# chilir/spotter

Hardware: AMD Instinct MI355X
Metric: images/sec RT-DETRv2-R101 640² bs32 at 1/2/4/8 MI355X; p50 /detect latency (higher is better)
Workload: dtype fp32; 1 GPU; RT-DETRv2-r101vd 640x640 batch=32/GPU preprocess+forward+postprocess; model=rtdetr_v2_r101vd, global_batch=32, image_size=640, parallelism=replicas x1

## Files before the change

### include/spotter_hip.h

```cpp
#ifndef SPOTTER_HIP_H
#define SPOTTER_HIP_H

#include <stddef.h>
#include <stdint.h>

#ifdef __cplusplus
extern "C" {
#endif

#define SP_ABI_VERSION 16

enum sp_act { SP_ACT_NONE = 0, SP_ACT_RELU = 1, SP_ACT_SILU = 2, SP_ACT_GELU = 3 };
enum sp_precision { SP_PREC_FP32 = 0, SP_PREC_BF16 = 1, SP_PREC_F32X3 = 2 };

typedef struct {
  const uint8_t* data;
  int32_t height, width;
  int32_t row_stride;
} sp_image_u8;

typedef struct {
  const float* A; int64_t lda;
  const float* A2; int64_t lda2;
  int32_t N, H, W, Cin;
  int32_t KH, KW, stride, pad;
  int32_t Ho, Wo;
  const float* Wt; int32_t Cout;
  const float* scale;
  const float* shift;
  const float* row_scale; int32_t row_period;
  const float* res1; int64_t ldr1;
  int32_t act;
  const float* res2; int64_t ldr2;
  float* C; int64_t ldc;
  int32_t out_rows_per_group; int64_t out_group_stride;
  float* workspace; int64_t workspace_elems;
  int32_t precision;
  const uint16_t* Wt_bf16;
  int64_t wt_plane_stride;
  const float* ln_gamma;
  const float* ln_beta;
  float ln_eps;
  const uint16_t* A_bf16;
  uint16_t* C_bf16;
  const uint16_t* res1_bf16;
  const uint16_t* res2_bf16;
  int32_t* splitk_counters; int64_t splitk_counters_len;
} sp_conv_desc;

typedef struct {
  const float* value; int64_t ld_value; int32_t value_col;
  const float* off_aw; int64_t ld_off_aw;
  const float* ref;
  float* out; int64_t ld_out;
  int32_t B, S, Q, heads, head_dim, levels, points;
  int32_t level_h[4], level_w[4], level_start[4];
  float offset_scale;
  const uint16_t* value_bf16;
} sp_msda_desc;

int sp_abi_version(void);
const char* sp_last_error(void);
enum sp_build_flag { SP_BUILD_FUSED_LN = 1, SP_BUILD_BOUNDS = 2 };
int sp_build_flags(void);
int64_t sp_bounds_report(char* buf, int64_t cap);
int sp_device_init(int device);
int sp_shutdown(void);

int sp_preprocess_u8(const sp_image_u8* images, int n, int out_h, int out_w, float* out,
                     void* stream);

int sp_conv2d(const sp_conv_desc* d, void* stream);
int sp_set_conv_config(int cfg);
int sp_set_splitk_config(int cfg, int max_splits, int min_ktiles);
enum sp_tuning_knob {
  SP_TUNE_GLDS_EPILOGUE = 3,
  SP_TUNE_MSDA_GENERIC = 4,
};
int sp_set_tuning(int knob, int value);

int sp_conv3x3_winograd(const sp_conv_desc* d, const uint16_t* wt_wino, int64_t wino_plane_stride, float* work,
                        int64_t work_elems, void* stream);
int sp_winograd_f23_input(const sp_conv_desc* d, float* work, int64_t work_elems, void* stream);
int sp_winograd_f23_gemm(const sp_conv_desc* d, const uint16_t* wt_wino, int64_t wino_plane_stride, float* work,
                         int64_t work_elems, void* stream);
int sp_winograd_f23_output(const sp_conv_desc* d, const float* work, int64_t work_elems, void* stream);
int sp_winograd_f43_input(const sp_conv_desc* d, float* work, int64_t work_elems, void* stream);
int sp_winograd_f43_gemm(const sp_conv_desc* d, const uint16_t* wt_wino, int64_t wino_plane_stride, float* work,
                         int64_t work_elems, void* stream);
int sp_winograd_f43_output(const sp_conv_desc* d, const float* work, int64_t work_elems, void* stream);

int sp_nchw_to_nhwc(const float* x, float* y, int n, int c, int h, int w, void* stream);
int sp_stem_conv3x3s2_nchw(const float* x, const float* wt, const float* scale, const float* shift, float* y,
                           int n, int h, int w, int cout, int act, void* stream);
int sp_stem_conv3x3s2_nchw_bf16(const float* x, const float* wt, const float* scale, const float* shift, uint16_t* y,
                                int n, int h, int w, int cout, int act, void* stream);
int sp_conv3x3_c32_bf16(const uint16_t* x, const uint16_t* w16, const float* scale, const float* shift, uint16_t* y,
                        int n, int h, int w, int cout, int act, void* stream);
int sp_conv3x3_c32(const float* x, const float* wt, const float* scale, const float* shift, float* y, int n, int h,
                   int w, int cout, int act, void* stream);
int sp_conv3x3_c64_bf16(const uint16_t* x, int64_t ldx, const uint16_t* w16, const float* scale, const float* shift,
                        uint16_t* y, int64_t ldy, const uint16_t* res, int64_t ldr, int n, int h, int w, int act,
                        void* stream);
int sp_maxpool3x3s2(const float* x, float* y, int64_t ldy, int n, int h, int w, int c, void* stream);
int sp_maxpool3x3s2_bf16(const uint16_t* x, uint16_t* y, int64_t ldy, int n, int h, int w, int c, void* stream);
int sp_avgpool2x2_ceil(const float* x, float* y, int64_t ldy, int n, int h, int w, int c, void* stream);
int sp_avgpool2x2_ceil_bf16(const uint16_t* x, uint16_t* y, int64_t ldy, int n, int h, int w, int c, void* stream);
int sp_upsample2x_nearest(const float* x, int64_t ldx, float* y, int64_t ldy, int n, int h,
                          int w, int c, void* stream);
int sp_layernorm(const float* x, int64_t ldx, const float* gamma, const float* beta, float* y,
                 int64_t ldy, int rows, int d, float eps, void* stream);
int sp_layernorm_bf16(const float* x, int64_t ldx, const float* gamma, const float* beta, uint16_t* y, int64_t ldy,
                      int rows, int d, float eps, void* stream);
int sp_attention(const float* q, int64_t ldq, const float* k, int64_t ldk, const float* v,
                 int64_t ldv, float* o, int64_t ldo, int batch, int n, int heads, int dh,
                 float scale, void* stream);
int sp_attention_bf16(const float* q, int64_t ldq, const float* k, int64_t ldk, const float* v,
                      int64_t ldv, float* o, int64_t ldo, int batch, int n, int heads, int dh,
                      float scale, void* stream);
int sp_msda(const sp_msda_desc* d, void* stream);
int sp_topk_rows(const float* x, int64_t ldx, int rows, int n, int reduce_c, int apply_sigmoid,
                 int k, float* vals, int32_t* idx, void* stream);
int sp_rowmax(const float* x, int64_t ldx, int64_t rows, int c, float* out, void* stream);
int sp_linear_rowmax_bf16(const uint16_t* a, int64_t lda, const uint16_t* w, const float* bias, int rows, int n,
                          int k, float* out, void* stream);
int sp_gather_rows(const float* src, int64_t ld_src, int src_rows, const int32_t* idx, int k,
                   int batch, int d, float* dst, int64_t ld_dst, void* stream);
int sp_add_rows(const float* a, int64_t lda, const float* b, int64_t ldb, float* y, uint16_t* y_bf16, int64_t ldy,
                int rows, int cols, void* stream);
int sp_ref_init(const float* delta, int64_t ld_delta, const float* anchors, const int32_t* idx,
                int batch, int k, float* ref, void* stream);
int sp_box_refine(const float* delta, int64_t ld_delta, float* ref, int rows, void* stream);
int sp_postprocess(const float* logits, const float* boxes, const int32_t* target_hw, int batch,
                   int q, int c, int k, float threshold, float* scores, int64_t* labels,
                   float* boxes_xyxy, int32_t* counts, int32_t* work, void* stream);

#define SP_JPEG_UNSUPPORTED (-10)
typedef struct {
  int32_t width, height;
  int32_t ncomp;
  int32_t color;
  int32_t progressive;
  int32_t max_h, max_v;
  int32_t h[3], v[3];
  int32_t bw[3], bh[3];
  int64_t block_off[3];
  int64_t total_blocks;
  int64_t plane_off[3];
  int64_t plane_bytes;
  uint16_t quant[3][64];
} sp_jpeg_layout;
int sp_jpeg_decode_coefs(const uint8_t* data, int64_t len, sp_jpeg_layout* lay, int16_t* coefs, int64_t coef_elems);
int sp_jpeg_to_rgb(const int16_t* coefs, const sp_jpeg_layout* lay, uint8_t* work, int64_t work_bytes, uint8_t* rgb,
                   int64_t rgb_stride, int32_t* status, void* stream);

typedef struct {
// ... 53 lines not shown
```

### spotter_amd/_lib.py

```python
from __future__ import annotations

import ctypes as C
import os
import threading

HERE = os.path.dirname(os.path.abspath(__file__))
LIB_PATH = os.environ.get("SPOTTER_HIP_LIB", os.path.join(HERE, "libspotter_hip.so"))
ABI_VERSION = 16

vp = C.c_void_p
i32 = C.c_int32
i64 = C.c_int64
f32 = C.c_float


class SpImageU8(C.Structure):
    _fields_ = [("data", vp), ("height", i32), ("width", i32), ("row_stride", i32)]


class SpConvDesc(C.Structure):
    _fields_ = [
        ("A", vp), ("lda", i64), ("A2", vp), ("lda2", i64),
        ("N", i32), ("H", i32), ("W", i32), ("Cin", i32),
        ("KH", i32), ("KW", i32), ("stride", i32), ("pad", i32),
        ("Ho", i32), ("Wo", i32),
        ("Wt", vp), ("Cout", i32),
        ("scale", vp), ("shift", vp),
        ("row_scale", vp), ("row_period", i32),
        ("res1", vp), ("ldr1", i64),
        ("act", i32),
        ("res2", vp), ("ldr2", i64),
        ("C", vp), ("ldc", i64),
        ("out_rows_per_group", i32), ("out_group_stride", i64),
        ("workspace", vp), ("workspace_elems", i64),
        ("precision", i32), ("Wt_bf16", vp), ("wt_plane_stride", i64),
        ("ln_gamma", vp), ("ln_beta", vp), ("ln_eps", f32),
        ("A_bf16", vp),
        ("C_bf16", vp), ("res1_bf16", vp), ("res2_bf16", vp),
        ("splitk_counters", vp), ("splitk_counters_len", i64),
    ]


class SpMsdaDesc(C.Structure):
    _fields_ = [
        ("value", vp), ("ld_value", i64), ("value_col", i32),
        ("off_aw", vp), ("ld_off_aw", i64),
        ("ref", vp),
        ("out", vp), ("ld_out", i64),
        ("B", i32), ("S", i32), ("Q", i32), ("heads", i32), ("head_dim", i32),
        ("levels", i32), ("points", i32),
        ("level_h", i32 * 4), ("level_w", i32 * 4), ("level_start", i32 * 4),
        ("offset_scale", f32),
        ("value_bf16", vp),
    ]


class SpJpegLayout(C.Structure):
    _fields_ = [
        ("width", i32), ("height", i32), ("ncomp", i32), ("color", i32), ("progressive", i32),
        ("max_h", i32), ("max_v", i32), ("h", i32 * 3), ("v", i32 * 3), ("bw", i32 * 3), ("bh", i32 * 3),
        ("block_off", i64 * 3), ("total_blocks", i64), ("plane_off", i64 * 3), ("plane_bytes", i64),
# ... 15 lines not shown
    _fields_ = [
        ("kind", i32), ("x0", i32), ("y0", i32), ("x1", i32), ("y1", i32), ("ink", C.c_uint32),
        ("mask_off", i64), ("mask_stride", i32), ("sx", i32), ("sy", i32), ("reserved", i32),
    ]


class SpDrawTile(C.Structure):
    _fields_ = [("tx", i32), ("ty", i32), ("first", i32), ("count", i32)]


class SpDrawTable(C.Structure):
    _fields_ = [
        ("n_ops", i32), ("n_tiles", i32), ("n_refs", i32), ("height", i32), ("width", i32), ("reserved", i32),
        ("ops_off", i64), ("tiles_off", i64), ("refs_off", i64), ("masks_off", i64), ("mask_bytes", i64),
        ("total_bytes", i64),
    ]


SP_DRAW_FILL, SP_DRAW_BLEND = 0, 1
SP_DRAW_TILE_W, SP_DRAW_TILE_H = 64, 8
SP_JPEG_UNSUPPORTED = -10
SP_BUILD_FUSED_LN = 1
SP_BUILD_BOUNDS = 2

_SIGS = {
    "sp_abi_version": (i32, []),
    "sp_build_flags": (i32, []),
    "sp_bounds_report": (i64, [C.c_char_p, i64]),
    "sp_last_error": (C.c_char_p, []),
    "sp_device_init": (i32, [i32]),
    "sp_shutdown": (i32, []),
    "sp_preprocess_u8": (i32, [C.POINTER(SpImageU8), i32, i32, i32, vp, vp]),
    "sp_conv2d": (i32, [C.POINTER(SpConvDesc), vp]),
    "sp_set_conv_config": (i32, [i32]),
    "sp_set_splitk_config": (i32, [i32, i32, i32]),
    "sp_set_tuning": (i32, [i32, i32]),
    "sp_conv3x3_winograd": (i32, [C.POINTER(SpConvDesc), vp, i64, vp, i64, vp]),
    "sp_winograd_f23_input": (i32, [C.POINTER(SpConvDesc), vp, i64, vp]),
    "sp_winograd_f23_gemm": (i32, [C.POINTER(SpConvDesc), vp, i64, vp, i64, vp]),
    "sp_winograd_f23_output": (i32, [C.POINTER(SpConvDesc), vp, i64, vp]),
    "sp_winograd_f43_input": (i32, [C.POINTER(SpConvDesc), vp, i64, vp]),
    "sp_winograd_f43_gemm": (i32, [C.POINTER(SpConvDesc), vp, i64, vp, i64, vp]),
    "sp_winograd_f43_output": (i32, [C.POINTER(SpConvDesc), vp, i64, vp]),
    "sp_nchw_to_nhwc": (i32, [vp, vp, i32, i32, i32, i32, vp]),
    "sp_stem_conv3x3s2_nchw": (i32, [vp, vp, vp, vp, vp, i32, i32, i32, i32, i32, vp]),
    "sp_maxpool3x3s2": (i32, [vp, vp, i64, i32, i32, i32, i32, vp]),
    "sp_avgpool2x2_ceil": (i32, [vp, vp, i64, i32, i32, i32, i32, vp]),
    "sp_maxpool3x3s2_bf16": (i32, [vp, vp, i64, i32, i32, i32, i32, vp]),
    "sp_avgpool2x2_ceil_bf16": (i32, [vp, vp, i64, i32, i32, i32, i32, vp]),
    "sp_stem_conv3x3s2_nchw_bf16": (i32, [vp, vp, vp, vp, vp, i32, i32, i32, i32, i32, vp]),
    "sp_conv3x3_c32_bf16": (i32, [vp, vp, vp, vp, vp, i32, i32, i32, i32, i32, vp]),
    "sp_conv3x3_c32": (i32, [vp, vp, vp, vp, vp, i32, i32, i32, i32, i32, vp]),
    "sp_conv3x3_c64_bf16": (i32, [vp, i64, vp, vp, vp, vp, i64, vp, i64, i32, i32, i32, i32, vp]),
    "sp_upsample2x_nearest": (i32, [vp, i64, vp, i64, i32, i32, i32, i32, vp]),
    "sp_layernorm": (i32, [vp, i64, vp, vp, vp, i64, i32, i32, f32, vp]),
    "sp_layernorm_bf16": (i32, [vp, i64, vp, vp, vp, i64, i32, i32, f32, vp]),
    "sp_attention": (i32, [vp, i64, vp, i64, vp, i64, vp, i64, i32, i32, i32, i32, f32, vp]),
    "sp_attention_bf16": (i32, [vp, i64, vp, i64, vp, i64, vp, i64, i32, i32, i32, i32, f32, vp]),
    "sp_msda": (i32, [C.POINTER(SpMsdaDesc), vp]),
    "sp_topk_rows": (i32, [vp, i64, i32, i32, i32, i32, i32, vp, vp, vp]),
    "sp_rowmax": (i32, [vp, i64, i64, i32, vp, vp]),
    "sp_gather_rows": (i32, [vp, i64, i32, vp, i32, i32, i32, vp, i64, vp]),
    "sp_ref_init": (i32, [vp, i64, vp, vp, i32, i32, vp, vp]),
    "sp_box_refine": (i32, [vp, i64, vp, i32, vp]),
    "sp_add_rows": (i32, [vp, i64, vp, i64, vp, vp, i64, i32, i32, vp]),
    "sp_linear_rowmax_bf16": (i32, [vp, i64, vp, vp, i32, i32, i32, vp, vp]),
    "sp_postprocess": (i32, [vp, vp, vp, i32, i32, i32, i32, f32, vp, vp, vp, vp, vp, vp]),
    "sp_jpeg_decode_coefs": (i32, [vp, i64, C.POINTER(SpJpegLayout), vp, i64]),
    "sp_jpeg_to_rgb": (i32, [vp, C.POINTER(SpJpegLayout), vp, i64, vp, i64, vp, vp]),
    "sp_jpeg_enc_plan": (i32, [i32, i32, i32, i32, C.POINTER(SpJpegEncLayout)]),
    "sp_jpeg_enc_rgb": (i32, [vp, i64, i32, C.POINTER(SpJpegEncLayout), vp, i64, vp, i64, vp, vp]),
    "sp_jpeg_enc_max_bytes": (i64, [C.POINTER(SpJpegEncLayout), i64, i64]),
    "sp_jpeg_enc_finish": (i32, [C.POINTER(SpJpegEncLayout), vp, i64, vp, i64, vp, i64, C.POINTER(i64)]),
    "sp_draw_pack": (i32, [vp, i32, vp, i64, i32, i32, vp, i64, C.POINTER(i64)]),
    "sp_draw_rgb": (i32, [vp, i32, i32, i64, vp, vp, i64, vp]),
}

EXPORTS = tuple(_SIGS)

_lock = threading.Lock()
_lib = None


def load(path: str = LIB_PATH):
    if not os.path.exists(path):
        raise RuntimeError(
            f"libspotter_hip.so not found at {path}; build it with `python -m spotter_amd.build_ext` "
            "(there is no CPU fallback)")
    import torch

    L = C.CDLL(path)
    for name, (res, args) in _SIGS.items():
        fn = getattr(L, name)
        fn.restype = res
        fn.argtypes = args
    if L.sp_abi_version() != ABI_VERSION:
        raise RuntimeError(f"libspotter_hip ABI {L.sp_abi_version()} != {ABI_VERSION}")
    return L


def lib():
    global _lib
    with _lock:
        if _lib is None:
            _lib = load()
        return _lib
# ... 11 lines not shown
```

### spotter_amd/engine.py

```python
from __future__ import annotations

import math

import numpy as np
import torch

from . import ops
from .config import PRECISIONS, SpotterConfig, check_precision
from .ops import V, view
from .weights import backbone_plan


def _t(a, dev):
    return torch.from_numpy(np.ascontiguousarray(a, dtype=np.float32)).to(dev)


bf16_bits = ops.bf16_bits


ATTN_BF16 = True

_X3_FASTER = {(256, 64, False), (256, 1024, True), (1024, 256, True), (512, 256, True), (256, 512, True),
              (288, 256, True), (4, 256, False)}



def _wkw(wq):
    if wq is None:
        return {}
    if wq.dim() == 2 and wq.shape[0] == 3:
        return {"wt_planes": wq}
    return {"wt16": wq}


class ConvW:
    __slots__ = ("w", "cin", "cout", "k", "scale", "shift", "w16", "host", "wino", "mode")

    def __init__(self, w, cin, cout, k, scale, shift, w16=None, host=None, mode="f32"):
        self.w, self.cin, self.cout, self.k, self.scale, self.shift = w, cin, cout, k, scale, shift
        self.w16 = w16
        self.mode = mode
        self.host = host
        self.wino = None


class LinW:
    __slots__ = ("w", "b", "k", "n", "w16", "mode")

    def __init__(self, w, b, k, n, w16=None, mode="f32"):
        self.w, self.b, self.k, self.n = w, b, k, n
        self.w16 = w16
        self.mode = mode


def frozen_bn_affine(p, pre):
    scale = p[pre + ".weight"] * (p[pre + ".running_var"] + np.float32(1e-5)) ** np.float32(-0.5)
    shift = p[pre + ".bias"] - p[pre + ".running_mean"] * scale
    return scale.astype(np.float32), shift.astype(np.float32)


def eval_bn_affine(p, pre, eps=1e-5):
    inv = (p[pre + ".running_var"] + np.float32(eps)) ** np.float32(-0.5)
    scale = p[pre + ".weight"] * inv
    shift = p[pre + ".bias"] - p[pre + ".running_mean"] * scale
    return scale.astype(np.float32), shift.astype(np.float32)


def conv_khwc(w):
    co, ci, k, _ = w.shape
    return np.ascontiguousarray(w.transpose(0, 2, 3, 1).reshape(co, k * k * ci))


def sine_pos_embed(h, w, dim, temperature):
    pd = dim // 4
    omega = 1.0 / temperature ** (np.arange(pd, dtype=np.float64) / pd)
    gh, gw = np.meshgrid(np.arange(h, dtype=np.float64), np.arange(w, dtype=np.float64), indexing="ij")
    eh = np.outer(gh.reshape(-1), omega)
    ew = np.outer(gw.reshape(-1), omega)
    return np.concatenate([np.sin(eh), np.cos(eh), np.sin(ew), np.cos(ew)], 1).astype(np.float32)


def anchors_for(shapes, grid_size=0.05):
    out = []
    f = np.float32
    for lvl, (h, w) in enumerate(shapes):
        gy, gx = np.meshgrid(np.arange(h, dtype=f), np.arange(w, dtype=f), indexing="ij")
        xy = np.stack([gx, gy], -1) + f(0.5)
        xy[..., 0] /= f(w)
        xy[..., 1] /= f(h)
        wh = np.ones_like(xy) * f(grid_size * 2.0 ** lvl)
        out.append(np.concatenate([xy, wh], -1).reshape(h * w, 4))
    a = np.concatenate(out, 0).astype(f)
    valid = ((a > f(1e-2)) & (a < f(1 - 1e-2))).all(-1)
    lg = np.log(a / (f(1) - a)).astype(f)
    lg[~valid] = np.finfo(f).max
    return lg, valid.astype(f)


class Engine:

    def __init__(self, cfg: SpotterConfig, weights: dict, device: str | torch.device = "cuda",
                 fold_repvgg: bool = True, precision: str = "fp32", fuse_shortcut: bool = True,
                 fuse_ln: bool = False, winograd: str | bool = "auto", wino_m: int = 4,
                 bf16_store: bool | None = None, direct_c32: bool = True,
                 direct_c64_bf16: bool = True, splitk_combine: bool = False):
        from ._lib import SP_BUILD_FUSED_LN, lib

        check_precision(precision)
        self.cfg = cfg
        self.fold_repvgg = fold_repvgg
        self.fuse_shortcut = fuse_shortcut
        self.fuse_ln = fuse_ln
        if fuse_ln and PRECISIONS.get(precision, ("", ""))[1] == "bf16":
            raise ValueError(f"fuse_ln=True runs the linears on fp32 weights: not available with precision={precision!r}")
        if fuse_ln and not (lib().sp_build_flags() & SP_BUILD_FUSED_LN):
            raise ValueError("fuse_ln=True needs a diagnostic library with the fused-LayerNorm tiles "
                             "(UNIT=conv_gemm tools/build_diag.sh <name> -DSP_DIAG_KERNELS=1; SPOTTER_HIP_LIB)")
        if winograd is True:
            winograd = "auto"
        if winograd not in (False, None, "auto", "repvgg", "all"):
            raise ValueError("winograd must be False, 'auto', 'repvgg' or 'all'")
        self.winograd = winograd or False
        if wino_m not in (2, 4):
            raise ValueError("wino_m must be 2 (F(2x2,3x3)) or 4 (F(4x4,3x3))")
        self.wino_m = wino_m
        self.precision = precision
        self.act_bb = cfg.hidden_act
        self.act_enc = cfg.activation_function
        self.act_aifi = cfg.encoder_activation_function
        self.act_dec = cfg.decoder_activation_function
        self._conv_mode, self._lin_mode = PRECISIONS[precision]
        self._attn_bf16 = self._lin_mode == "bf16" and ATTN_BF16
        self.bf16_store = (self._conv_mode == "bf16") if bf16_store is None else bool(bf16_store)
        if self.bf16_store and self._conv_mode != "bf16":
            raise ValueError("bf16_store needs a bf16 conv operand mode")
        self.direct_c32 = direct_c32
        self.direct_c64_bf16 = direct_c64_bf16
        self.splitk_combine = splitk_combine
        self.splitk_min_rows = 0
        self.add_rows = True
        self.enc_head_bf16 = True
        self.enc_rowmax_fused = True
        self.dev = torch.device(device)
        if self.dev.type != "cuda":
            raise RuntimeError("spotter_amd runs on an MI355X (gfx950) device only")
        idx = self.dev.index if self.dev.index is not None else torch.cuda.current_device()
        self.dev = torch.device("cuda", idx)
        rc = lib().sp_device_init(idx)
        if rc != 0:
            raise RuntimeError(f"sp_device_init: {lib().sp_last_error().decode()}")
        with torch.cuda.device(self.dev):
            self._pack(weights)
        self._ws = {}
        self._consts = {}
        self._ctxs = {}
        self._outs = {}
        self.microbatches = None
        self.stagger = 1

    def _wq(self, w: np.ndarray, mode: str):
        if mode == "f32":
            return None
        if mode == "bf16":
            return torch.from_numpy(bf16_bits(w).view(np.int16)).to(self.dev)
        return torch.from_numpy(ops.split_bf16x3_host(w)).to(self.dev)

    def _add_wino(self, cw: ConvW):
        if cw.k != 3 or cw.mode == "f32" or cw.cin % 32 or cw.cout % 4 or not self.winograd:
            return cw
        if self.winograd == "auto" and (cw.cin < (self.WINO43_MIN_CIN if self.wino_m == 4 else 256) or cw.mode != "x3"):
            return cw
        u = ops.winograd_weights_host(cw.host.reshape(cw.cout, 3, 3, cw.cin), self.wino_m)
        if cw.mode == "x3":
            cw.wino = torch.from_numpy(ops.split_bf16x3_host(u)).to(self.dev)
        else:
            cw.wino = torch.from_numpy(bf16_bits(u).reshape(1, -1).view(np.int16)).to(self.dev)
        return cw

    def _pick(self, mode: str, cout: int, kdim: int, small_m: bool = False) -> str:
        if mode == "x3" and self.precision == "fp32" and (cout <= 64 or kdim <= 64 or small_m):
            if cout == 64 and kdim >= 576 and not small_m:
                return mode
            if (cout, kdim, small_m) in _X3_FASTER:
                return mode
            return "f32"
        return mode

    def _mk_conv(self, wk, ci, co, k, sc, sh):
        wk = np.ascontiguousarray(wk, dtype=np.float32)
        mode = self._pick(self._conv_mode, co, ci * k * k)
        return ConvW(_t(wk, self.dev), ci, co, k, _t(sc, self.dev), _t(sh, self.dev), self._wq(wk, mode), host=wk,
                     mode=mode)

    def _conv(self, p, conv_key, bn_pre, frozen):
        w = p[conv_key]
        co, ci, k, _ = w.shape
        sc, sh = frozen_bn_affine(p, bn_pre) if frozen else eval_bn_affine(p, bn_pre, self.cfg.batch_norm_eps)
        return self._mk_conv(conv_khwc(w), ci, co, k, sc, sh)

    def _lin(self, p, pre, *more, per_query: bool = False):
        ws = [p[pre + ".weight"]] + [p[m + ".weight"] for m in more]
        bs = [p[pre + ".bias"]] + [p[m + ".bias"] for m in more]
        w = np.ascontiguousarray(np.concatenate(ws, 0))
        b = np.concatenate(bs, 0)
        wd = _t(w, self.dev)
        mode = self._pick(self._lin_mode, w.shape[0], w.shape[1], small_m=per_query and w.shape[0] > 128)
        return LinW(wd, _t(b, self.dev), w.shape[1], w.shape[0], self._wq(w.astype(np.float32), mode), mode=mode)

    def _ln(self, p, pre):
        return (_t(p[pre + ".weight"], self.dev), _t(p[pre + ".bias"], self.dev))

    def _pack(self, p):
        cfg = self.cfg
        bb = "model.backbone.model"
        self.stem = [self._conv(p, f"{bb}.embedder.embedder.{i}.convolution.weight",
                                f"{bb}.embedder.embedder.{i}.normalization", True) for i in range(3)]
        self.blocks = []
        for (s, i, lt, cin, cout, st, sc) in backbone_plan(cfg):
            pre = f"{bb}.encoder.stages.{s}.layers.{i}"
            blk = {"s": s, "i": i, "type": lt, "cin": cin, "cout": cout, "stride": st, "sc": sc}
            if sc == "conv":
                blk["short"] = self._conv(p, pre + ".shortcut.convolution.weight", pre + ".shortcut.normalization", True)
            elif sc == "avgconv":
                blk["short"] = self._conv(p, pre + ".shortcut.1.convolution.weight", pre + ".shortcut.1.normalization", True)
            nl = 3 if lt == "bottleneck" else 2
            blk["layers"] = [self._conv(p, f"{pre}.layer.{j}.convolution.weight", f"{pre}.layer.{j}.normalization", True)
                             for j in range(nl)]
            if self.winograd in ("auto", "all"):
                for j, c in enumerate(blk["layers"]):
                    if c.k == 3 and (st == 1 or (lt != "bottleneck" and j == 1)):
                        self._add_wino(c)
            if self.fuse_shortcut and lt == "bottleneck" and (sc == "avgconv" or (sc == "conv" and st == 1)):
                sk = pre + (".shortcut.1" if sc == "avgconv" else ".shortcut")
                blk["fused"] = self._fused_tail(p, f"{pre}.layer.2", sk, cin)
            self.blocks.append(blk)
        self.in_proj = [self._conv(p, f"model.encoder_input_proj.{l}.0.weight", f"model.encoder_input_proj.{l}.1", False)
                        for l in range(len(cfg.encoder_in_channels))]
        a = "model.encoder.aifi.0.layers.0"
        self.aifi = {
            "qk": self._lin(p, a + ".self_attn.q_proj", a + ".self_attn.k_proj"),
            "v": self._lin(p, a + ".self_attn.v_proj"),
            "o": self._lin(p, a + ".self_attn.o_proj"),
            "ln1": self._ln(p, a + ".self_attn_layer_norm"),
            "fc1": self._lin(p, a + ".mlp.fc1"),
            "fc2": self._lin(p, a + ".mlp.fc2"),
            "ln2": self._ln(p, a + ".final_layer_norm"),
        }
        E = "model.encoder"
        nl = len(cfg.encoder_in_channels)
        self.lateral = [self._conv(p, f"{E}.lateral_convs.{i}.conv.weight", f"{E}.lateral_convs.{i}.norm", False)
                        for i in range(nl - 1)]
        self.down = [self._conv(p, f"{E}.downsample_convs.{i}.conv.weight", f"{E}.downsample_convs.{i}.norm", False)
                     for i in range(nl - 1)]
        self.fpn = [self._csp(p, f"{E}.fpn_blocks.{i}") for i in range(nl - 1)]
        self.pan = [self._csp(p, f"{E}.pan_blocks.{i}") for i in range(nl - 1)]
        self.dec_proj = [self._conv(p, f"model.decoder_input_proj.{l}.0.weight", f"model.decoder_input_proj.{l}.1", False)
                         for l in range(len(cfg.decoder_in_channels))]
        self.enc_output = self._lin(p, "model.enc_output.0")
        self.enc_ln = self._ln(p, "model.enc_output.1")
        self.enc_score = self._lin(p, "model.enc_score_head")
        self.enc_bbox = [self._lin(p, f"model.enc_bbox_head.layers.{i}", per_query=True) for i in range(3)]
        self.qpos = [self._lin(p, f"model.decoder.query_pos_head.layers.{i}", per_query=True) for i in range(2)]
        D = "model.decoder.layers"
        L = cfg.decoder_layers
        self.value_all = self._lin(p, f"{D}.0.encoder_attn.value_proj",
                                   *[f"{D}.{j}.encoder_attn.value_proj" for j in range(1, L)])
        self.dec = []
        for j in range(L):
            q = f"{D}.{j}"
# ... 50 lines not shown
                reps.append((self._conv(p, q + ".conv1.conv.weight", q + ".conv1.norm", False),
                             self._conv(p, q + ".conv2.conv.weight", q + ".conv2.norm", False)))
        c3 = None
        if (pre + ".conv3.conv.weight") in p:
            c3 = self._conv(p, pre + ".conv3.conv.weight", pre + ".conv3.norm", False)
        return {"c12": c12, "hid": w1.shape[0], "reps": reps, "c3": c3}

    def _buf(self, key, *shape, dtype=torch.float32):
        ws = self._ws
        t = ws.get(key)
        n = int(np.prod(shape))
        if t is None or t.numel() < n or t.dtype != dtype:
            t = torch.empty(n, dtype=dtype, device=self.dev)
            ws[key] = t
        return t[:n]

    SPLITK_COUNTERS = 4096

    def _splitk(self) -> dict:
        kw = {"workspace": self._buf("splitk", self.SPLITK_ELEMS)}
        if self.splitk_combine:
            c = self._ws.get("splitk_cnt")
            if c is None:
                c = torch.zeros(self.SPLITK_COUNTERS, dtype=torch.int32, device=self.dev)
                self._ws["splitk_cnt"] = c
            kw["counters"] = c
        return kw

    def _const(self, key, fn):
        c = self._consts.get(key)
        if c is None:
            c = fn()
            self._consts[key] = c
        return c

    SPLITK_ELEMS = 16 << 20
    WINO43_MIN_CIN = 128
    WINO_MIN_PIXELS = 8192
    WINO43_MIN_WORK = 1 << 19

    def _wino_pays(self, pixels: int, cin: int) -> bool:
        if self.wino_m == 4:
            return pixels * cin >= self.WINO43_MIN_WORK and (cin >= self.WINO43_MIN_CIN or self.winograd != "auto")
        return pixels >= self.WINO_MIN_PIXELS

    def _cv(self, x: V, n, h, w, cw: ConvW, stride, out: V, act=None, res1=None, res2=None, **kw):
        pad = cw.k // 2
        if (cw.cin == 64 and cw.cout == 64 and cw.k == 3 and stride == 1 and not kw and res2 is None
                and act in ("relu", None) and n * h * w >= self.C64_MIN_PIXELS):
            rows16 = lambda v: v.ld % 8 == 0 and v.off % 8 == 0
            if (self.direct_c64_bf16 and x.is_bf16 and out.is_bf16 and cw.mode == "bf16" and rows16(x)
                    and rows16(out) and (res1 is None or (res1.is_bf16 and rows16(res1)))):
                return ops.conv3x3_c64_bf16(x, cw.w16, cw.scale, cw.shift, out, n, h, w, act=act, res1=res1)
        if cw.wino is not None and stride == 1 and not kw and not x.is_bf16 and self._wino_pays(n * h * w, cw.cin):
            wm = self.wino_m
            tiles = n * ((h + wm - 1) // wm) * ((w + wm - 1) // wm)
            work = self._buf("wino_work", ops.wino_work_elems(wm, tiles, cw.cin, cw.cout))
            return ops.conv2d(x, n, h, w, cw.cin, cw.w, cw.cout, 3, 1, 1, out, scale=cw.scale, shift=cw.shift,
                              act=act, res1=res1, res2=res2, wino=(cw.wino, work, wm))
        return ops.conv2d(x, n, h, w, cw.cin, cw.w, cw.cout, cw.k, stride, pad, out, scale=cw.scale,
                          shift=cw.shift, act=act, res1=res1, res2=res2,
                          **self._splitk(), **_wkw(cw.w16), **kw)

    def _lin_op(self, x: V, rows, lw: LinW, out: V, act=None, res1=None, res2=None, a2=None, row_scale=None,
                ln=None):
        if ln is not None and self.fuse_ln:
            if act is not None or res2 is not None:
                raise ValueError("fused LayerNorm epilogue: act / res2 are not implemented")
            if lw.mode == "bf16":
                raise ValueError("fuse_ln runs fp32 weights: not available on a bf16-operand layer")
            return ops.linear(x, rows, lw.k, lw.w, lw.n, out, bias=lw.b, res1=res1, a2=a2, row_scale=row_scale,
                              ln=(ln[0], ln[1], self.cfg.layer_norm_eps))
        if ln is not None:
            tmp = view(self._buf("ln_tmp", rows, lw.n), lw.n)
            ops.linear(x, rows, lw.k, lw.w, lw.n, tmp, bias=lw.b, act=act, res1=res1, res2=res2, a2=a2,
                       row_scale=row_scale, **self._splitk(), **_wkw(lw.w16))
            return ops.layernorm(tmp, *ln, out, rows, lw.n, self.cfg.layer_norm_eps)
        sk = self._splitk() if rows > self.splitk_min_rows else {}
        return ops.linear(x, rows, lw.k, lw.w, lw.n, out, bias=lw.b, act=act, res1=res1, res2=res2, a2=a2,
                          row_scale=row_scale, **sk, **_wkw(lw.w16))

    def _lin_plus(self, x: V, addend: V | None, rows, lw: LinW, out: V, key: str):
        if addend is None:
            return self._lin_op(x, rows, lw, out)
        if not self.add_rows or lw.mode == "f32":
            return self._lin_op(x, rows, lw, out, a2=addend)
        hp = view(self._buf(key, rows, lw.k, dtype=torch.int16 if lw.mode == "bf16" else torch.float32), lw.k)
        ops.add_rows(x, addend, hp, rows, lw.k)
        return self._lin_op(hp, rows, lw, out)

    C64_MIN_PIXELS = 1 << 18
    C32_MIN_PIXELS = 1 << 19

    def _direct_stem(self) -> bool:
        c = self.stem[0]
        return c.cin == 3 and c.k == 3 and c.cout in (32, 64) and self.act_bb in ("relu", None)

    def backbone(self, pixel_values: torch.Tensor, B, H, W):
        e = self.cfg.embedding_size
        h1, w1 = (H - 1) // 2 + 1, (W - 1) // 2 + 1
        dt = torch.int16 if self.bf16_store else torch.float32

        def buf(key, *shape):
            return self._buf(key, *shape, dtype=dt)

        s0 = buf("stem0", B, h1, w1, e // 2)
        s1 = buf("stem1", B, h1, w1, e // 2)
        s2 = buf("stem2", B, h1, w1, e)
        c0 = self.stem[0]
        if self._direct_stem():
            ops.stem_conv_nchw(pixel_values, c0.w, c0.scale, c0.shift, view(s0, e // 2), c0.cout, act=self.act_bb)
        else:
            px = self._buf("px_nhwc", B, H, W, 3)
            ops.nchw_to_nhwc(pixel_values, px)
            self._cv(view(px, 3), B, H, W, c0, 2, view(s0, e // 2), act=self.act_bb)
        for src, cw, dst in ((s0, self.stem[1], s1), (s1, self.stem[2], s2)):
            c32 = cw.cin == 32 and cw.k == 3 and cw.cout in (32, 64) and self.act_bb in ("relu", None)
            if c32 and self.bf16_store:
                ops.conv3x3_c32_bf16(view(src, cw.cin), cw.w16, cw.scale, cw.shift, view(dst, cw.cout), B, h1, w1,
                                     cw.cout, act=self.act_bb)
            elif (c32 and self.direct_c32 and cw.mode == "f32" and not self.bf16_store
                  and B * h1 * w1 >= self.C32_MIN_PIXELS):
                ops.conv3x3_c32(view(src, cw.cin), cw.w, cw.scale, cw.shift, view(dst, cw.cout), B, h1, w1, cw.cout,
                                act=self.act_bb)
            else:
                self._cv(view(src, cw.cin), B, h1, w1, cw, 1, view(dst, cw.cout), act=self.act_bb)
        h, w = (h1 - 1) // 2 + 1, (w1 - 1) // 2 + 1
        b0 = self.blocks[0]
        if "fused" in b0 and b0["sc"] == "conv":
            kc = b0["layers"][0].cout + e
            curv = V(buf(f"s{b0['s']}_cat", B, h, w, kc), kc - e, kc)
        else:
            curv = view(buf("pool", B, h, w, e), e)
        ops.maxpool3x3s2(s2, curv, B, h1, w1, e)
        c = e
        feats = []
        nstage = len(self.cfg.depths)
        for blk in self.blocks:
            s, i, st, cout = blk["s"], blk["i"], blk["stride"], blk["cout"]
            cur = curv.t
            if i == 0 and s > 0:
                assert curv.off == 0 and curv.ld == c
                feats.append((cur, h, w, c))
            ho, wo = (h - 1) // st + 1, (w - 1) // st + 1
            L = blk["layers"]
            if "fused" in blk:
                red = L[0].cout
                kc = red + c
                if blk["sc"] == "avgconv":
                    assert curv.off == 0 and curv.ld == c
                    cat = buf(f"s{s}_cat", B, ho, wo, kc)
                    ops.avgpool2x2_ceil(cur, V(cat, red, kc), B, h, w, c)
                else:
                    assert curv.off == red and curv.ld == kc and st == 1
                    cat = cur
                t1 = buf(f"s{s}_t1", B, h, w, red)
                out = buf(f"s{s}_out{i % 2}", B, ho, wo, cout)
                self._cv(curv, B, h, w, L[0], 1, view(t1, red), act=self.act_bb)
                self._cv(view(t1, red), B, h, w, L[1], st, V(cat, 0, kc), act=self.act_bb)
                self._cv(V(cat, 0, kc), B, ho, wo, blk["fused"], 1, view(out, cout), act=self.act_bb)
                curv, h, w, c = view(out, cout), ho, wo, cout
                yield
                continue
            if blk["sc"] == "identity":
                res = view(cur, c)
            else:
                src, sh_, sw_ = cur, h, w
                if blk["sc"] == "avgconv":
                    pooled = buf(f"s{s}_pool", B, (h + 1) // 2, (w + 1) // 2, c)
                    ops.avgpool2x2_ceil(cur, pooled, B, h, w, c)
                    src, sh_, sw_ = pooled, (h + 1) // 2, (w + 1) // 2
                sbuf = buf(f"s{s}_sc", B, ho, wo, cout)
                self._cv(view(src, c), B, sh_, sw_, blk["short"], 1 if blk["sc"] == "avgconv" else st, view(sbuf, cout))
# ... 279 lines not shown
```

### spotter_amd/ops.py

```python
from __future__ import annotations

import ctypes as C
from dataclasses import dataclass

import numpy as np
import torch

from ._lib import SpConvDesc, SpImageU8, SpMsdaDesc, call

ACT = {None: 0, "none": 0, "relu": 1, "silu": 2, "gelu": 3}

_hook = None


def set_launch_hook(hook):
    global _hook
    _hook = hook


def _launch(kind: str, name: str, args, flops: int = 0, nbytes: int = 0, shape=None):
    if _hook is None:
        call(name, *args)
    else:
        _hook(kind, lambda: call(name, *args), flops, nbytes, shape)
# ... 263 lines not shown
            (x.data_ptr(), wt.data_ptr(), scale.data_ptr(), shift.data_ptr(), yp, n, h, w, cout, ACT[act],
             stream()), 2 * m * cout * 27, 4 * (x.numel() + cout * 27) + y.t.element_size() * m * cout,
            (m, cout, 27, 3, 2, "direct"))
    return ho, wo


def conv3x3_c32_bf16(x: V, w16: torch.Tensor, scale: torch.Tensor, shift: torch.Tensor, y: V, n: int, h: int,
                     w: int, cout: int, act=None):
    if not (x.is_bf16 and y.is_bf16) or x.ld != 32 or y.ld != cout or x.off % 8 or y.off % 8:
        raise ValueError("conv3x3_c32_bf16: dense bf16 rows (ld 32 in, Cout out) expected")
    if w16.dtype != torch.int16 or w16.numel() != cout * 288 or scale.numel() < cout or shift.numel() < cout:
        raise ValueError("conv3x3_c32_bf16: weight / affine size mismatch")
    m = n * h * w
    xp = x.need(m, 32, "c32.x", bf16=True)
    yp = y.need(m, cout, "c32.y", bf16=True)
    _launch("conv", "sp_conv3x3_c32_bf16", (xp, w16.data_ptr(), scale.data_ptr(), shift.data_ptr(), yp, n, h, w,
                                            cout, ACT[act], stream()),
            2 * m * cout * 288, 2 * (m * 32 + cout * 288 + m * cout), (m, cout, 288, 3, 1, "bf16-direct"))


def conv3x3_c32(x: V, wt: torch.Tensor, scale: torch.Tensor, shift: torch.Tensor, y: V, n: int, h: int, w: int,
                cout: int, act=None):
    if x.is_bf16 or y.is_bf16 or x.ld != 32 or y.ld != cout:
        raise ValueError("conv3x3_c32: dense fp32 rows (ld 32 in, Cout out) expected")
    if wt.dtype != torch.float32 or wt.numel() != cout * 288 or scale.numel() < cout or shift.numel() < cout:
        raise ValueError("conv3x3_c32: weight / affine size mismatch")
    m = n * h * w
    xp = x.need(m, 32, "c32.x")
    yp = y.need(m, cout, "c32.y")
    _launch("conv", "sp_conv3x3_c32", (xp, wt.data_ptr(), scale.data_ptr(), shift.data_ptr(), yp, n, h, w, cout,
                                       ACT[act], stream()),
            2 * m * cout * 288, 4 * (m * 32 + cout * 288 + m * cout), (m, cout, 288, 3, 1, "f32-direct"))


def conv3x3_c64_bf16(x: V, w16: torch.Tensor, scale: torch.Tensor, shift: torch.Tensor, y: V, n: int, h: int,
                     w: int, act=None, res1: V | None = None):
    if not (x.is_bf16 and y.is_bf16) or x.ld % 8 or x.off % 8 or y.ld % 8 or y.off % 8:
        raise ValueError("conv3x3_c64_bf16: 16-byte aligned bf16 row views expected")
    if w16.dtype != torch.int16 or w16.numel() != 64 * 576 or scale.numel() < 64 or shift.numel() < 64:
        raise ValueError("conv3x3_c64_bf16: weight / affine size mismatch")
    m = n * h * w
    xp = x.need(m, 64, "c64b.x", bf16=True)
    yp = y.need(m, 64, "c64b.y", bf16=True)
    rp, ldr = None, 0
    if res1 is not None:
        if not res1.is_bf16 or res1.ld % 8 or res1.off % 8:
            raise ValueError("conv3x3_c64_bf16: the residual must be 16-byte aligned bf16 rows")
        rp, ldr = res1.need(m, 64, "c64b.res", bf16=True), res1.ld
    _launch("conv", "sp_conv3x3_c64_bf16", (xp, x.ld, w16.data_ptr(), scale.data_ptr(), shift.data_ptr(), yp, y.ld,
                                            rp, ldr, n, h, w, ACT[act], stream()),
            2 * m * 64 * 576, 2 * (m * 64 + 64 * 576 + m * 64 * (2 if rp else 1)), (m, 64, 576, 3, 1, "bf16-direct"))


def _pool_out(y, m: int, c: int, what: str):
    if isinstance(y, V):
        if y.ld % 4 or y.off % 4 or (y.is_bf16 and (y.ld % 8 or y.off % 8)):
            raise ValueError(f"{what}: output view must be 16-byte aligned")
        return y.need(m, c, what, bf16=y.is_bf16), y.ld
    if y.numel() < m * c:
        raise ValueError(f"{what}: output too small")
    return y.data_ptr(), c


def _pool(name, x: torch.Tensor, y, n, h, w, c, ho, wo):
    assert x.numel() >= n * h * w * c
    bf = x.dtype == torch.int16
    yv = y if isinstance(y, V) else view(y, c)
    if yv.is_bf16 != bf:
        raise TypeError(f"{name}: input and output rows must both be float32 or both bf16")
    yp, ldy = _pool_out(y, n * ho * wo, c, name + ".y")
    _launch("elementwise", name + ("_bf16" if bf else ""), (x.data_ptr(), yp, ldy, n, h, w, c, stream()), 0,
            x.element_size() * n * c * (h * w + ho * wo))
    return ho, wo


def maxpool3x3s2(x: torch.Tensor, y, n, h, w, c):
    return _pool("sp_maxpool3x3s2", x, y, n, h, w, c, (h - 1) // 2 + 1, (w - 1) // 2 + 1)


def avgpool2x2_ceil(x: torch.Tensor, y, n, h, w, c):
    return _pool("sp_avgpool2x2_ceil", x, y, n, h, w, c, (h + 1) // 2, (w + 1) // 2)


def upsample2x(x: V, y: V, n, h, w, c):
    bf = x.is_bf16
    if y.is_bf16 != bf:
        raise TypeError("upsample: input and output rows must both be float32 or both bf16")
    xp = x.need(n * h * w, c, "upsample.x", bf16=bf)
    yp = y.need(n * 4 * h * w, c, "upsample.y", bf16=bf)
    if bf and (c % 8 or x.ld % 2 or y.ld % 2 or x.off % 2 or y.off % 2):
        raise ValueError("upsample: bf16 rows need c % 8 == 0 and even strides / offsets")
    k = 2 if bf else 1
    _launch("elementwise", "sp_upsample2x_nearest", (xp, x.ld // k, yp, y.ld // k, n, h, w, c // k, stream()), 0,
            x.t.element_size() * n * h * w * c * 5)


def layernorm(x: V, gamma, beta, y: V, rows, d, eps=1e-5):
    xp = x.need(rows, d, "ln.x")
    yp = y.need(rows, d, "ln.y", bf16=y.is_bf16)
    _launch("layernorm", "sp_layernorm_bf16" if y.is_bf16 else "sp_layernorm",
            (xp, x.ld, gamma.data_ptr(), beta.data_ptr(), yp, y.ld, rows, d, eps, stream()), 8 * rows * d,
            (4 + y.t.element_size()) * rows * d)


def attention(q: V, k: V, v: V, o: V, batch, n, heads, dh, scale, bf16: bool = False):
    rows = batch * n
# ... 117 lines not shown
```

Baseline: 810.3 images/sec.

## Add direct 3x3 conv kernels using split-bf16x3 MFMA for fp32 c64/c32 layers

Adds a direct (implicit-GEMM) 3x3 conv kernel that splits fp32 activations into three bf16 planes in LDS and runs six bf16 MFMA products per fragment to emulate fp32 accuracy. It tiles 8x32 output pixels with a halo, double-buffers weights with async global-to-LDS loads, and prefetches the next tile's halo into registers. The 64-channel variant is enabled by default for x3-mode convs without a residual, replacing the previous GEMM or Winograd path. The 32-channel stem variant is behind a flag that is off by default. It trades im2col and workspace traffic for extra MFMA work and a persistent grid of one block per CU, and the x3 split approximates fp32 rather than matching it exactly.

```diff
diff --git a/include/spotter_hip.h b/include/spotter_hip.h
--- a/include/spotter_hip.h
+++ b/include/spotter_hip.h
@@ -8,7 +8,7 @@
 extern "C" {
 #endif
 
-#define SP_ABI_VERSION 16
+#define SP_ABI_VERSION 17
 
 enum sp_act { SP_ACT_NONE = 0, SP_ACT_RELU = 1, SP_ACT_SILU = 2, SP_ACT_GELU = 3 };
 enum sp_precision { SP_PREC_FP32 = 0, SP_PREC_BF16 = 1, SP_PREC_F32X3 = 2 };
@@ -102,6 +102,10 @@
 int sp_conv3x3_c64_bf16(const uint16_t* x, int64_t ldx, const uint16_t* w16, const float* scale, const float* shift,
                         uint16_t* y, int64_t ldy, const uint16_t* res, int64_t ldr, int n, int h, int w, int act,
                         void* stream);
+int sp_conv3x3_c64_x3(const float* x, int64_t ldx, const uint16_t* w_planes, int64_t plane_stride, const float* scale,
+                      const float* shift, float* y, int64_t ldy, int n, int h, int w, int act, void* stream);
+int sp_conv3x3_c32_x3(const float* x, const uint16_t* w_planes, int64_t plane_stride, const float* scale,
+                      const float* shift, float* y, int n, int h, int w, int cout, int act, void* stream);
 int sp_maxpool3x3s2(const float* x, float* y, int64_t ldy, int n, int h, int w, int c, void* stream);
 int sp_maxpool3x3s2_bf16(const uint16_t* x, uint16_t* y, int64_t ldy, int n, int h, int w, int c, void* stream);
 int sp_avgpool2x2_ceil(const float* x, float* y, int64_t ldy, int n, int h, int w, int c, void* stream);
diff --git a/spotter_amd/_lib.py b/spotter_amd/_lib.py
--- a/spotter_amd/_lib.py
+++ b/spotter_amd/_lib.py
@@ -6,7 +6,7 @@
 
 HERE = os.path.dirname(os.path.abspath(__file__))
 LIB_PATH = os.environ.get("SPOTTER_HIP_LIB", os.path.join(HERE, "libspotter_hip.so"))
-ABI_VERSION = 16
+ABI_VERSION = 17
 
 vp = C.c_void_p
 i32 = C.c_int32
@@ -128,6 +128,8 @@
     "sp_conv3x3_c32_bf16": (i32, [vp, vp, vp, vp, vp, i32, i32, i32, i32, i32, vp]),
     "sp_conv3x3_c32": (i32, [vp, vp, vp, vp, vp, i32, i32, i32, i32, i32, vp]),
     "sp_conv3x3_c64_bf16": (i32, [vp, i64, vp, vp, vp, vp, i64, vp, i64, i32, i32, i32, i32, vp]),
+    "sp_conv3x3_c64_x3": (i32, [vp, i64, vp, i64, vp, vp, vp, i64, i32, i32, i32, i32, vp]),
+    "sp_conv3x3_c32_x3": (i32, [vp, vp, i64, vp, vp, vp, i32, i32, i32, i32, i32, vp]),
     "sp_upsample2x_nearest": (i32, [vp, i64, vp, i64, i32, i32, i32, i32, vp]),
     "sp_layernorm": (i32, [vp, i64, vp, vp, vp, i64, i32, i32, f32, vp]),
     "sp_layernorm_bf16": (i32, [vp, i64, vp, vp, vp, i64, i32, i32, f32, vp]),
diff --git a/spotter_amd/csrc/direct_x3.hip b/spotter_amd/csrc/direct_x3.hip
--- /dev/null
+++ b/spotter_amd/csrc/direct_x3.hip
@@ -0,0 +1,214 @@
+#include "mfma16_common.h"
+
+namespace sp {
+namespace {
+
+constexpr int DX_TH = 8, DX_TW = 32, DX_HR = DX_TH + 2, DX_HC = DX_TW + 2, DX_NPX = DX_HR * DX_HC;
+
+template <int CIN, int CO, bool RES>
+__global__ __launch_bounds__(512, 1) void conv3x3_x3_kernel(const float* __restrict__ x,
+                                                            const uint16_t* __restrict__ wp, int64_t wps,
+                                                            const float* __restrict__ scale,
+                                                            const float* __restrict__ shift, float* __restrict__ y,
+                                                            int64_t ldx, int64_t ldy, int nimg, int h, int w,
+                                                            int tiles_x, int tiles_y, int act) {
+  constexpr int CPP = CIN / 8;
+  constexpr int PLANE = DX_NPX * CPP;
+  constexpr int SPT = CIN / 32;
+  constexpr int NST = 9 * SPT;
+  constexpr int WPL = CO * 4;
+  constexpr int WST = 3 * WPL;
+  constexpr int NBUF = RES ? NST : 2;
+  constexpr int WDMA = WST / 64;
+  constexpr int TMN = CO / 32;
+  constexpr int PFN = (PLANE + 511) / 512;
+  __shared__ uint4 lds[3 * PLANE + NBUF * WST];
+  __shared__ float aff[2 * CO];
+  uint4* halo = lds;
+  uint4* wl = lds + 3 * PLANE;
+  const int tid = threadIdx.x, lane = tid & 63;
+  const int wave = __builtin_amdgcn_readfirstlane(tid >> 6);
+  auto hswz = [](int col, int c) { return CIN == 64 ? c ^ ((col >> 1) & 7) : c ^ ((col >> 2) & 3); };
+  if (tid < CO) {
+    aff[tid] = scale[tid];
+    aff[CO + tid] = shift[tid];
+  }
+  const uint32_t wl0 = (uint32_t)(uintptr_t)(__attribute__((address_space(3))) uint4*)wl;
+  auto issue_w = [&](int st, int buf) {
+#pragma unroll
+    for (int jj = 0; jj < (WDMA + 7) / 8; ++jj) {
+      const int j = wave + 8 * jj;
+      if (j < WDMA) {
+        const int idx = j * 64 + lane;
+        const int pl = idx / WPL, rem = idx - pl * WPL, n = rem >> 2, q = rem & 3;
+        const int64_t off = pl * wps + (int64_t)n * (9 * CIN) + st * 32 + ((q ^ ((n >> 2) & 3)) * 8);
+        SP_BCHECK(off + 7, 3 * wps);
+        glds16(wp + off, wl0 + (uint32_t)((buf * WST + j * 64) * 16));
+      }
+    }
+  };
+  const int64_t ntiles = (int64_t)nimg * tiles_x * tiles_y;
+  float4 pf[PFN][2];
+  unsigned okm = 0;
+  auto fetch = [&](int64_t t) {
+    const int tx = (int)(t % tiles_x);
+    t /= tiles_x;
+    const int ty = (int)(t % tiles_y);
+    const int b = (int)(t / tiles_y);
+    SP_BCHECK(b, nimg);
+    const int oy0 = ty * DX_TH, ox0 = tx * DX_TW;
+#pragma unroll
+    for (int k = 0; k < PFN; ++k) {
+      const int i = tid + k * 512;
+      const int c = i % CPP, rc = i / CPP, r = rc / DX_HC, col = rc - r * DX_HC;
+      const int iy = oy0 - 1 + r, ix = ox0 - 1 + col;
+      const bool ok = i < PLANE && (unsigned)iy < (unsigned)h && (unsigned)ix < (unsigned)w;
+      const int64_t off = ok ? (((int64_t)b * h + iy) * w + ix) * ldx + c * 8 : 0;
+      SP_BCHECK(off + 7, ((int64_t)nimg * h * w - 1) * ldx + CIN);
+      pf[k][0] = *reinterpret_cast<const float4*>(x + off);
+      pf[k][1] = *reinterpret_cast<const float4*>(x + off + 4);
+      okm = k == 0 ? (unsigned)ok : (okm | ((unsigned)ok << k));
+    }
+  };
+  auto stash = [&]() {
+#pragma unroll
+    for (int k = 0; k < PFN; ++k) {
+      const int i = tid + k * 512;
+      if (i < PLANE) {
+        const int c = i % CPP, rc = i / CPP, col = rc % DX_HC;
+        const bool ok = (okm >> k) & 1u;
+        const float4 z = make_float4(0.f, 0.f, 0.f, 0.f);
+        bf16x8 pl[3];
+        split_frag_pk<3>(ok ? pf[k][0] : z, ok ? pf[k][1] : z, pl);
+        const int pos = rc * CPP + hswz(col, c);
+#pragma unroll
+        for (int q = 0; q < 3; ++q) halo[q * PLANE + pos] = __builtin_bit_cast(uint4, pl[q]);
+      }
+    }
+  };
+  if constexpr (RES) {
+#pragma unroll
+    for (int st = 0; st < NST; ++st) issue_w(st, st);
+  } else {
+    issue_w(0, 0);
+  }
+  if ((int64_t)blockIdx.x < ntiles) fetch(blockIdx.x);
+  const int r = lane & 31, hh = lane >> 5;
+  int par = 0;
+
+  for (int64_t tile = blockIdx.x; tile < ntiles; tile += gridDim.x) {
+    __syncthreads();
+    stash();
+    int64_t t = tile;
+    const int tx = (int)(t % tiles_x);
+    t /= tiles_x;
+    const int ty = (int)(t % tiles_y);
+    const int b = (int)(t / tiles_y);
+    SP_BCHECK(b, nimg);
+    const int oy = ty * DX_TH + wave, ox = tx * DX_TW + r;
+    f32x16 acc[TMN];
+#pragma unroll
+    for (int i = 0; i < TMN; ++i)
+#pragma unroll
+      for (int q = 0; q < 16; ++q) acc[i][q] = 0.f;
+#pragma unroll
+    for (int st = 0; st < NST; ++st) {
+      const int buf = RES ? st : (st + par) & 1;
+      if (!RES || st == 0) {
+        wait_vmcnt<0>();
+        __syncthreads();
+      }
+      if constexpr (!RES) issue_w(st + 1 < NST ? st + 1 : 0, buf ^ 1);
+      if (st == 0 && tile + gridDim.x < ntiles) fetch(tile + gridDim.x);
+      const int tap = st / SPT, cq = st - tap * SPT, kh = tap / 3, kw = tap - 3 * kh;
+      const uint4* wb = wl + buf * WST;
+      const int col = r + kw;
+      const uint4* hp = halo + ((wave + kh) * DX_HC + col) * CPP;
+#pragma unroll
+      for (int s2 = 0; s2 < 2; ++s2) {
+        const int chw = 2 * s2 + hh;
+        bf16x8 xa[3], wf[TMN][3];
+#pragma unroll
+        for (int q = 0; q < 3; ++q) xa[q] = *reinterpret_cast<const bf16x8*>(hp + q * PLANE + hswz(col, cq * 4 + chw));
+#pragma unroll
+        for (int i = 0; i < TMN; ++i) {
+          const int n = i * 32 + r;
+#pragma unroll
+          for (int q = 0; q < 3; ++q)
+            wf[i][q] = *reinterpret_cast<const bf16x8*>(wb + q * WPL + n * 4 + (chw ^ ((n >> 2) & 3)));
+        }
+#pragma unroll
+        for (int i = 0; i < TMN; ++i) {
+          acc[i] = __builtin_amdgcn_mfma_f32_32x32x16_bf16(wf[i][0], xa[2], acc[i], 0, 0, 0);
+          acc[i] = __builtin_amdgcn_mfma_f32_32x32x16_bf16(wf[i][2], xa[0], acc[i], 0, 0, 0);
+          acc[i] = __builtin_amdgcn_mfma_f32_32x32x16_bf16(wf[i][1], xa[1], acc[i], 0, 0, 0);
+          acc[i] = __builtin_amdgcn_mfma_f32_32x32x16_bf16(wf[i][0], xa[1], acc[i], 0, 0, 0);
+          acc[i] = __builtin_amdgcn_mfma_f32_32x32x16_bf16(wf[i][1], xa[0], acc[i], 0, 0, 0);
+          acc[i] = __builtin_amdgcn_mfma_f32_32x32x16_bf16(wf[i][0], xa[0], acc[i], 0, 0, 0);
+        }
+      }
+    }
+    if constexpr (!RES) par = (par + NST) & 1;
+    if (oy < h && ox < w) {
+      const int64_t pix = ((int64_t)b * h + oy) * w + ox;
+      SP_BCHECK(pix, (int64_t)nimg * h * w);
+      float* yrow = y + pix * ldy;
+#pragma unroll
+      for (int i = 0; i < TMN; ++i)
+#pragma unroll
+        for (int g = 0; g < 4; ++g) {
+          const int n0 = i * 32 + 8 * g + 4 * hh;
+          float4 v;
+          float* vv = &v.x;
+#pragma unroll
+          for (int e = 0; e < 4; ++e) {
+            const float u = fmaf(acc[i][4 * g + e], aff[n0 + e], aff[CO + n0 + e]);
+            vv[e] = act ? fmaxf(u, 0.f) : u;
+          }
+          *reinterpret_cast<float4*>(yrow + n0) = v;
+        }
+    }
+  }
+  wait_vmcnt<0>();
+}
+
+template <int CIN, int CO, bool RES>
+int dx_launch(const char* what, const float* x, int64_t ldx, const uint16_t* wp, int64_t wps, const float* scale,
+              const float* shift, float* y, int64_t ldy, int n, int h, int w, int act, void* stream) {
+  const int tiles_x = (w + DX_TW - 1) / DX_TW, tiles_y = (h + DX_TH - 1) / DX_TH;
+  const int64_t tiles = (int64_t)n * tiles_x * tiles_y;
+  const unsigned grid = (unsigned)(tiles < g_num_cus ? tiles : g_num_cus);
+  hipLaunchKernelGGL((conv3x3_x3_kernel<CIN, CO, RES>), dim3(grid), dim3(512), 0, as_stream(stream), x, wp, wps,
+                     scale, shift, y, ldx, ldy, n, h, w, tiles_x, tiles_y, act);
+  return check_launch(what);
+}
+
+}
+}
+
+extern "C" int sp_conv3x3_c64_x3(const float* x, int64_t ldx, const uint16_t* w_planes, int64_t plane_stride,
+                                 const float* scale, const float* shift, float* y, int64_t ldy, int n, int h, int w,
+                                 int act, void* stream) {
+  using namespace sp;
+  SP_ARG_CHECK(x && w_planes && scale && shift && y && n > 0 && h > 0 && w > 0 && (act == 0 || act == 1) &&
+                   ldx >= 64 && ldy >= 64 && ldx % 4 == 0 && ldy % 4 == 0 && plane_stride >= 64 * 576 &&
+                   plane_stride % 8 == 0 && ((uintptr_t)x & 15) == 0 && ((uintptr_t)w_planes & 15) == 0 &&
+                   ((uintptr_t)y & 15) == 0,
+               "sp_conv3x3_c64_x3: bad args (act none/relu, 16-byte aligned fp32 rows, ld % 4, ld >= 64, planes [3][64][576])");
+  return dx_launch<64, 64, false>("sp_conv3x3_c64_x3", x, ldx, w_planes, plane_stride, scale, shift, y, ldy, n, h, w,
+                                  act, stream);
+}
+
+extern "C" int sp_conv3x3_c32_x3(const float* x, const uint16_t* w_planes, int64_t plane_stride, const float* scale,
+                                 const float* shift, float* y, int n, int h, int w, int cout, int act, void* stream) {
+  using namespace sp;
+  SP_ARG_CHECK(x && w_planes && scale && shift && y && n > 0 && h > 0 && w > 0 && (cout == 32 || cout == 64) &&
+                   (act == 0 || act == 1) && plane_stride >= (int64_t)cout * 288 && plane_stride % 8 == 0 &&
+                   ((uintptr_t)x & 15) == 0 && ((uintptr_t)w_planes & 15) == 0 && ((uintptr_t)y & 15) == 0,
+               "sp_conv3x3_c32_x3: bad args (Cin 32, Cout 32 or 64, act none/relu, aligned dense fp32 rows, planes [3][Cout][288])");
+  if (cout == 32)
+    return dx_launch<32, 32, true>("sp_conv3x3_c32_x3", x, 32, w_planes, plane_stride, scale, shift, y, 32, n, h, w, act,
+                                   stream);
+  return dx_launch<32, 64, false>("sp_conv3x3_c32_x3", x, 32, w_planes, plane_stride, scale, shift, y, 64, n, h, w, act,
+                                  stream);
+}
diff --git a/spotter_amd/engine.py b/spotter_amd/engine.py
--- a/spotter_amd/engine.py
+++ b/spotter_amd/engine.py
@@ -34,7 +34,7 @@
 
 
 class ConvW:
-    __slots__ = ("w", "cin", "cout", "k", "scale", "shift", "w16", "host", "wino", "mode")
+    __slots__ = ("w", "cin", "cout", "k", "scale", "shift", "w16", "host", "wino", "mode", "x3p")
 
     def __init__(self, w, cin, cout, k, scale, shift, w16=None, host=None, mode="f32"):
         self.w, self.cin, self.cout, self.k, self.scale, self.shift = w, cin, cout, k, scale, shift
@@ -42,6 +42,7 @@
         self.mode = mode
         self.host = host
         self.wino = None
+        self.x3p = None
 
 
 class LinW:
@@ -103,7 +104,8 @@
                  fold_repvgg: bool = True, precision: str = "fp32", fuse_shortcut: bool = True,
                  fuse_ln: bool = False, winograd: str | bool = "auto", wino_m: int = 4,
                  bf16_store: bool | None = None, direct_c32: bool = True,
-                 direct_c64_bf16: bool = True, splitk_combine: bool = False):
+                 direct_c64_bf16: bool = True, splitk_combine: bool = False, direct_c64_x3: bool = True,
+                 direct_c32_x3: bool = False):
         from ._lib import SP_BUILD_FUSED_LN, lib
 
         check_precision(precision)
@@ -136,6 +138,8 @@
             raise ValueError("bf16_store needs a bf16 conv operand mode")
         self.direct_c32 = direct_c32
         self.direct_c64_bf16 = direct_c64_bf16
+        self.direct_c64_x3 = direct_c64_x3
+        self.direct_c32_x3 = direct_c32_x3
         self.splitk_combine = splitk_combine
         self.splitk_min_rows = 0
         self.add_rows = True
@@ -215,6 +219,10 @@
         bb = "model.backbone.model"
         self.stem = [self._conv(p, f"{bb}.embedder.embedder.{i}.convolution.weight",
                                 f"{bb}.embedder.embedder.{i}.normalization", True) for i in range(3)]
+        if self.precision == "fp32" and self._conv_mode == "x3" and self.direct_c32_x3:
+            for cw in self.stem[1:]:
+                if cw.cin == 32 and cw.k == 3 and cw.cout in (32, 64) and cw.mode == "f32":
+                    cw.x3p = torch.from_numpy(ops.split_bf16x3_host(cw.host)).to(self.dev)
         self.blocks = []
         for (s, i, lt, cin, cout, st, sc) in backbone_plan(cfg):
             pre = f"{bb}.encoder.stages.{s}.layers.{i}"
@@ -371,6 +379,9 @@
             if (self.direct_c64_bf16 and x.is_bf16 and out.is_bf16 and cw.mode == "bf16" and rows16(x)
                     and rows16(out) and (res1 is None or (res1.is_bf16 and rows16(res1)))):
                 return ops.conv3x3_c64_bf16(x, cw.w16, cw.scale, cw.shift, out, n, h, w, act=act, res1=res1)
+            rows4 = lambda v: not v.is_bf16 and v.ld % 4 == 0 and v.off % 4 == 0
+            if self.direct_c64_x3 and cw.mode == "x3" and res1 is None and rows4(x) and rows4(out):
+                return ops.conv3x3_c64_x3(x, cw.w16, cw.scale, cw.shift, out, n, h, w, act=act)
         if cw.wino is not None and stride == 1 and not kw and not x.is_bf16 and self._wino_pays(n * h * w, cw.cin):
             wm = self.wino_m
             tiles = n * ((h + wm - 1) // wm) * ((w + wm - 1) // wm)
@@ -438,6 +449,10 @@
             if c32 and self.bf16_store:
                 ops.conv3x3_c32_bf16(view(src, cw.cin), cw.w16, cw.scale, cw.shift, view(dst, cw.cout), B, h1, w1,
                                      cw.cout, act=self.act_bb)
+            elif (c32 and self.direct_c32_x3 and cw.x3p is not None and self.precision == "fp32"
+                  and B * h1 * w1 >= self.C32_MIN_PIXELS):
+                ops.conv3x3_c32_x3(view(src, cw.cin), cw.x3p, cw.scale, cw.shift, view(dst, cw.cout), B, h1, w1,
+                                   cw.cout, act=self.act_bb)
             elif (c32 and self.direct_c32 and cw.mode == "f32" and not self.bf16_store
                   and B * h1 * w1 >= self.C32_MIN_PIXELS):
                 ops.conv3x3_c32(view(src, cw.cin), cw.w, cw.scale, cw.shift, view(dst, cw.cout), B, h1, w1, cw.cout,
diff --git a/spotter_amd/ops.py b/spotter_amd/ops.py
--- a/spotter_amd/ops.py
+++ b/spotter_amd/ops.py
@@ -339,6 +339,43 @@
             2 * m * 64 * 576, 2 * (m * 64 + 64 * 576 + m * 64 * (2 if rp else 1)), (m, 64, 576, 3, 1, "bf16-direct"))
 
 
+def _x3_planes(wt_planes: torch.Tensor, numel: int, what: str):
+    if (wt_planes.dim() != 2 or wt_planes.shape[0] != 3 or wt_planes.shape[1] != numel
+            or wt_planes.dtype != torch.int16 or not wt_planes.is_contiguous() or not wt_planes.is_cuda):
+        raise ValueError(f"{what}: weight planes must be a contiguous int16 CUDA tensor [3, {numel}]")
+    return wt_planes.data_ptr(), wt_planes.shape[1]
+
+
+def conv3x3_c64_x3(x: V, wt_planes: torch.Tensor, scale: torch.Tensor, shift: torch.Tensor, y: V, n: int, h: int,
+                   w: int, act=None):
+    if x.is_bf16 or y.is_bf16 or x.ld % 4 or x.off % 4 or y.ld % 4 or y.off % 4:
+        raise ValueError("conv3x3_c64_x3: 16-byte aligned fp32 row views expected")
+    if scale.numel() < 64 or shift.numel() < 64 or ACT[act] > 1:
+        raise ValueError("conv3x3_c64_x3: affine size / activation (none or relu)")
+    wp, wps = _x3_planes(wt_planes, 64 * 576, "conv3x3_c64_x3")
+    m = n * h * w
+    xp = x.need(m, 64, "c64x3.x")
+    yp = y.need(m, 64, "c64x3.y")
+    _launch("conv", "sp_conv3x3_c64_x3", (xp, x.ld, wp, wps, scale.data_ptr(), shift.data_ptr(), yp, y.ld, n, h, w,
+                                          ACT[act], stream()),
+            2 * m * 64 * 576, 4 * (m * 64 + m * 64) + 6 * 64 * 576, (m, 64, 576, 3, 1, "x3", "direct"))
+
+
+def conv3x3_c32_x3(x: V, wt_planes: torch.Tensor, scale: torch.Tensor, shift: torch.Tensor, y: V, n: int, h: int,
+                   w: int, cout: int, act=None):
+    if x.is_bf16 or y.is_bf16 or x.ld != 32 or y.ld != cout or x.off % 4 or y.off % 4 or cout not in (32, 64):
+        raise ValueError("conv3x3_c32_x3: dense fp32 rows (ld 32 in, Cout 32 or 64 out) expected")
+    if scale.numel() < cout or shift.numel() < cout or ACT[act] > 1:
+        raise ValueError("conv3x3_c32_x3: affine size / activation (none or relu)")
+    wp, wps = _x3_planes(wt_planes, cout * 288, "conv3x3_c32_x3")
+    m = n * h * w
+    xp = x.need(m, 32, "c32x3.x")
+    yp = y.need(m, cout, "c32x3.y")
+    _launch("conv", "sp_conv3x3_c32_x3", (xp, wp, wps, scale.data_ptr(), shift.data_ptr(), yp, n, h, w, cout,
+                                          ACT[act], stream()),
+            2 * m * cout * 288, 4 * (m * 32 + m * cout) + 6 * cout * 288, (m, cout, 288, 3, 1, "x3", "direct"))
+
+
 def _pool_out(y, m: int, c: int, what: str):
     if isinstance(y, V):
         if y.ld % 4 or y.off % 4 or (y.is_bf16 and (y.ld % 8 or y.off % 8)):
```

Result: faster. 822.8 images/sec (median of 6 runs) (+1.5%).
